# xdspacelab/openvslam

Measured on AMD Instinct MI355X. Metric: ORB kpts+descriptors/sec and Hamming matches/sec @1920x1080, 8-level pyramid, higher is better.
Workload: dtype u8; 1 GPU; BASELINE configs[1]: 1920x1080 mono, 8 pyramid levels (x1.2), 2000 ORB features, extract + robust::brute_force_match (thr 50, ratio 0.9) against the previous frame; distinct_input_batches=2

## Files before the change

openvslam_amd/csrc/orb_describe.hip:

```cpp
#include <cstdlib>

#include "ovs_common.h"

namespace ovs {

__constant__ int8_t c_pattern[256 * 4] = {
#include "orb_pattern.inc"
};
__constant__ int32_t c_umax[16] = {15, 15, 15, 15, 14, 14, 14, 13, 13, 12, 11, 10, 9, 8, 6, 3};
__constant__ uint32_t c_ic_tab[16 * 2 * 8] = {
    0x01010100u, 0x01010101u, 0x01010101u, 0x01010101u, 0x03020100u, 0x07060504u, 0x0b0a0908u, 0x0f0e0d0cu,
    0x01010101u, 0x01010101u, 0x01010101u, 0x01010101u, 0x13121110u, 0x17161514u, 0x1b1a1918u, 0x1f1e1d1cu,
    0x01010100u, 0x01010101u, 0x01010101u, 0x01010101u, 0x03020100u, 0x07060504u, 0x0b0a0908u, 0x0f0e0d0cu,
    0x01010101u, 0x01010101u, 0x01010101u, 0x01010101u, 0x13121110u, 0x17161514u, 0x1b1a1918u, 0x1f1e1d1cu,
    0x01010100u, 0x01010101u, 0x01010101u, 0x01010101u, 0x03020100u, 0x07060504u, 0x0b0a0908u, 0x0f0e0d0cu,
    0x01010101u, 0x01010101u, 0x01010101u, 0x01010101u, 0x13121110u, 0x17161514u, 0x1b1a1918u, 0x1f1e1d1cu,
    0x01010100u, 0x01010101u, 0x01010101u, 0x01010101u, 0x03020100u, 0x07060504u, 0x0b0a0908u, 0x0f0e0d0cu,
    0x01010101u, 0x01010101u, 0x01010101u, 0x01010101u, 0x13121110u, 0x17161514u, 0x1b1a1918u, 0x1f1e1d1cu,
    0x01010000u, 0x01010101u, 0x01010101u, 0x01010101u, 0x03020000u, 0x07060504u, 0x0b0a0908u, 0x0f0e0d0cu,
    0x01010101u, 0x01010101u, 0x01010101u, 0x00010101u, 0x13121110u, 0x17161514u, 0x1b1a1918u, 0x001e1d1cu,
    0x01010000u, 0x01010101u, 0x01010101u, 0x01010101u, 0x03020000u, 0x07060504u, 0x0b0a0908u, 0x0f0e0d0cu,
    0x01010101u, 0x01010101u, 0x01010101u, 0x00010101u, 0x13121110u, 0x17161514u, 0x1b1a1918u, 0x001e1d1cu,
    0x01010000u, 0x01010101u, 0x01010101u, 0x01010101u, 0x03020000u, 0x07060504u, 0x0b0a0908u, 0x0f0e0d0cu,
    0x01010101u, 0x01010101u, 0x01010101u, 0x00010101u, 0x13121110u, 0x17161514u, 0x1b1a1918u, 0x001e1d1cu,
    0x01000000u, 0x01010101u, 0x01010101u, 0x01010101u, 0x03000000u, 0x07060504u, 0x0b0a0908u, 0x0f0e0d0cu,
    0x01010101u, 0x01010101u, 0x01010101u, 0x00000101u, 0x13121110u, 0x17161514u, 0x1b1a1918u, 0x00001d1cu,
    0x01000000u, 0x01010101u, 0x01010101u, 0x01010101u, 0x03000000u, 0x07060504u, 0x0b0a0908u, 0x0f0e0d0cu,
    0x01010101u, 0x01010101u, 0x01010101u, 0x00000101u, 0x13121110u, 0x17161514u, 0x1b1a1918u, 0x00001d1cu,
    0x00000000u, 0x01010101u, 0x01010101u, 0x01010101u, 0x00000000u, 0x07060504u, 0x0b0a0908u, 0x0f0e0d0cu,
    0x01010101u, 0x01010101u, 0x01010101u, 0x00000001u, 0x13121110u, 0x17161514u, 0x1b1a1918u, 0x0000001cu,
    0x00000000u, 0x01010100u, 0x01010101u, 0x01010101u, 0x00000000u, 0x07060500u, 0x0b0a0908u, 0x0f0e0d0cu,
    0x01010101u, 0x01010101u, 0x01010101u, 0x00000000u, 0x13121110u, 0x17161514u, 0x1b1a1918u, 0x00000000u,
    0x00000000u, 0x01010000u, 0x01010101u, 0x01010101u, 0x00000000u, 0x07060000u, 0x0b0a0908u, 0x0f0e0d0cu,
    0x01010101u, 0x01010101u, 0x00010101u, 0x00000000u, 0x13121110u, 0x17161514u, 0x001a1918u, 0x00000000u,
    0x00000000u, 0x01000000u, 0x01010101u, 0x01010101u, 0x00000000u, 0x07000000u, 0x0b0a0908u, 0x0f0e0d0cu,
    0x01010101u, 0x01010101u, 0x00000101u, 0x00000000u, 0x13121110u, 0x17161514u, 0x00001918u, 0x00000000u,
    0x00000000u, 0x00000000u, 0x01010101u, 0x01010101u, 0x00000000u, 0x00000000u, 0x0b0a0908u, 0x0f0e0d0cu,
    0x01010101u, 0x01010101u, 0x00000001u, 0x00000000u, 0x13121110u, 0x17161514u, 0x00000018u, 0x00000000u,
    0x00000000u, 0x00000000u, 0x01010000u, 0x01010101u, 0x00000000u, 0x00000000u, 0x0b0a0000u, 0x0f0e0d0cu,
    0x01010101u, 0x00010101u, 0x00000000u, 0x00000000u, 0x13121110u, 0x00161514u, 0x00000000u, 0x00000000u,
    0x00000000u, 0x00000000u, 0x00000000u, 0x01010100u, 0x00000000u, 0x00000000u, 0x00000000u, 0x0f0e0d00u,
    0x01010101u, 0x00000000u, 0x00000000u, 0x00000000u, 0x13121110u, 0x00000000u, 0x00000000u, 0x00000000u,
};
constexpr uint32_t kG0123 = 18u | (34u << 8) | (48u << 16) | (56u << 24);
constexpr uint32_t kG456 = 48u | (34u << 8) | (18u << 16);
constexpr uint32_t kG0123Indep = 18u | (34u << 8) | (49u << 16) | (55u << 24);
constexpr uint32_t kG456Indep = 49u | (34u << 8) | (18u << 16);

constexpr int kPatch = 43;
constexpr int kPatchR = 21;
constexpr int kBlurW = 37;
constexpr int kBlurR = 18;
constexpr int kPatchPitch = 64;
constexpr int kHbPitch = 40;
static_assert(kBlurW <= kHbPitch && kBlurW + 6 == kPatch, "blur window geometry");

__device__ __forceinline__ float fast_atan2_deg(float y, float x) {
    const float p1 = 0.9997878412794807f * (float)(180 / 3.14159265358979323846);
    const float p3 = -0.3258083974640975f * (float)(180 / 3.14159265358979323846);
    const float p5 = 0.1555786518463281f * (float)(180 / 3.14159265358979323846);
    const float p7 = -0.04432655554792128f * (float)(180 / 3.14159265358979323846);
    const float eps = 2.2204460492503131e-16f;
    const float ax = fabsf(x), ay = fabsf(y);
    float a, c, c2;
    if (ax >= ay) {
        c = __fdiv_rn(ay, __fadd_rn(ax, eps));
        c2 = __fmul_rn(c, c);
        a = __fmul_rn(__fadd_rn(__fmul_rn(__fadd_rn(__fmul_rn(__fadd_rn(__fmul_rn(p7, c2), p5), c2), p3), c2), p1), c);
    } else {
        c = __fdiv_rn(ax, __fadd_rn(ay, eps));
        c2 = __fmul_rn(c, c);
        a = __fsub_rn(90.f, __fmul_rn(__fadd_rn(__fmul_rn(__fadd_rn(__fmul_rn(__fadd_rn(__fmul_rn(p7, c2), p5), c2), p3), c2), p1), c));
    }
    if (x < 0) a = __fsub_rn(180.f, a);
    if (y < 0) a = __fsub_rn(360.f, a);
    return a;
}

__device__ __forceinline__ float poly_cos(float v) {
    const float c1 = 0.99940307f, c2 = -0.49558072f, c3 = 0.03679168f;
    const float v2 = __fmul_rn(v, v);
    return __fadd_rn(c1, __fmul_rn(v2, __fadd_rn(c2, __fmul_rn(c3, v2))));
}
__device__ __forceinline__ float util_cos(float v) {
    const float kPi = 3.14159265358979323846f, kTwoPi = 6.28318530717958647692f, kHalfPi = 1.57079632679489661923f,
                kThreeHalfPi = 4.71238898038468985769f, kInvTwoPi = 0.15915494309189533577f;
    v = __fsub_rn(v, __fmul_rn(floorf(__fmul_rn(v, kInvTwoPi)), kTwoPi));
    v = (0.0f < v) ? v : -v;
    if (v < kHalfPi) return poly_cos(v);
    if (v < kPi) return -poly_cos(__fsub_rn(kPi, v));
    if (v < kThreeHalfPi) return -poly_cos(__fsub_rn(v, kPi));
    return poly_cos(__fsub_rn(kTwoPi, v));
}
__device__ __forceinline__ float util_sin(float v) { return util_cos(__fsub_rn(1.57079632679489661923f, v)); }

template <int BYTE>
__device__ __forceinline__ float cvt_s8(uint32_t w) {
    float f;
    if (BYTE == 0) asm("v_cvt_f32_i32_sdwa %0, sext(%1) dst_sel:DWORD dst_unused:UNUSED_PAD src0_sel:BYTE_0" : "=v"(f) : "v"(w));
    if (BYTE == 1) asm("v_cvt_f32_i32_sdwa %0, sext(%1) dst_sel:DWORD dst_unused:UNUSED_PAD src0_sel:BYTE_1" : "=v"(f) : "v"(w));
    if (BYTE == 2) asm("v_cvt_f32_i32_sdwa %0, sext(%1) dst_sel:DWORD dst_unused:UNUSED_PAD src0_sel:BYTE_2" : "=v"(f) : "v"(w));
    if (BYTE == 3) asm("v_cvt_f32_i32_sdwa %0, sext(%1) dst_sel:DWORD dst_unused:UNUSED_PAD src0_sel:BYTE_3" : "=v"(f) : "v"(w));
    return f;
}

__device__ __forceinline__ int wave_total_in_lane63(int v) {
    v += __builtin_amdgcn_update_dpp(0, v, 0x111, 0xf, 0xf, true);
    v += __builtin_amdgcn_update_dpp(0, v, 0x112, 0xf, 0xf, true);
    v += __builtin_amdgcn_update_dpp(0, v, 0x114, 0xf, 0xf, true);
    v += __builtin_amdgcn_update_dpp(0, v, 0x118, 0xf, 0xf, true);
    v += __builtin_amdgcn_update_dpp(0, v, 0x142, 0xa, 0xf, false);
    v += __builtin_amdgcn_update_dpp(0, v, 0x143, 0xc, 0xf, false);
    return v;
}

__global__ __launch_bounds__(64) void k_describe(const FrameGeo* __restrict__ geo, const uint8_t* __restrict__ img0, size_t stride0,
                                                size_t frame_stride0, const uint8_t* __restrict__ pyr, size_t pyr_frame_bytes,
                                                const uint64_t* __restrict__ lvl_kps, const uint32_t* __restrict__ lvl_count,
                                                ovs_keypoint* __restrict__ kps, uint8_t* __restrict__ desc,
                                                int32_t* __restrict__ counts, int cap, int batch, ovs_keypoint* __restrict__ kps_m,
                                                uint8_t* __restrict__ desc_m, int32_t* __restrict__ counts_m) {
    __shared__ __attribute__((aligned(16))) uint8_t patch[kPatch * kPatchPitch];
    __shared__ __attribute__((aligned(16))) uint16_t hblur[kPatch * kHbPitch];

    const int lane = threadIdx.x;
    const int total_cap = geo->total_kp_cap;
    const uint32_t xcd = blockIdx.x & 7u, idx = blockIdx.x >> 3;
    const uint32_t grp = idx / (uint32_t)total_cap;
    const int kslot = (int)(idx - grp * (uint32_t)total_cap);
    const int frame = (int)(grp * 8u + xcd);
    if (frame >= batch) return;
    const int L = geo->num_levels;
    int level = 0;
    for (int l = 1; l < L; ++l)
        if (kslot >= geo->lv[l].kp_base) level = l;
    const LevelGeo& g = geo->lv[level];
    const int slot = kslot - g.kp_base;
    const uint32_t* cnt = lvl_count + frame * L;
    if (kslot == 0 && lane == 0) {
        int total = 0;
        for (int l = 0; l < L; ++l) total += cnt[l];
        counts[frame] = total < cap ? total : cap;
        if (counts_m) counts_m[frame] = total < cap ? total : cap;
    }
    if (slot >= (int)cnt[level]) return;
    int out_idx = slot;
    for (int l = 0; l < level; ++l) out_idx += cnt[l];
    if (out_idx >= cap) return;

    const uint64_t kp = lvl_kps[(size_t)frame * total_cap + kslot];
    const int x = (int)cand_x(kp), y = (int)cand_y(kp);
    const uint8_t* img;
    int pitch;
    if (level == 0) {
        img = img0 + (size_t)frame * frame_stride0;
        pitch = (int)stride0;
    } else {
        img = pyr + (size_t)frame * pyr_frame_bytes + g.plane_off;
        pitch = g.pitch;
    }
    const int xs = x - kPatchR;
    const int xa = xs & ~15;
    const int off = __builtin_amdgcn_readfirstlane(xs - xa);
    const uint8_t* seg0 = img + (size_t)(y - kPatchR) * pitch + xa;
    if (((pitch & 15) == 0) && ((reinterpret_cast<uintptr_t>(img) & 15) == 0)) {
#pragma unroll
        for (int j = 0; j < 3; ++j) {
            const int i = lane + 64 * j;
            if (i < kPatch * 4) {
                const int r = i >> 2, q = i & 3;
                *reinterpret_cast<uint4*>(patch + r * kPatchPitch + 16 * q) = *reinterpret_cast<const uint4*>(seg0 + (size_t)r * pitch + 16 * q);
            }
        }
    } else {
        for (int i = lane; i < kPatch * 16; i += 64) {
            const int r = i >> 4, q = i & 15;
            *reinterpret_cast<uint32_t*>(patch + r * kPatchPitch + 4 * q) = *reinterpret_cast<const uint32_t*>(seg0 + (size_t)r * pitch + 4 * q);
        }
    }
    __syncthreads();

    int m10 = 0, m01 = 0;
    if (lane < 62) {
        const int v = (lane >> 1) - 15, h = lane & 1;
        const int first = off + kPatchR + (h ? 0 : -16);
        const uint32_t* pw = reinterpret_cast<const uint32_t*>(patch + (kPatchR + v) * kPatchPitch + (first & ~3));
        const int shb = first & 3;
        const uint32_t w0 = pw[0], w1 = pw[1], w2 = pw[2], w3 = pw[3], w4 = pw[4];
        const uint32_t px[4] = {__builtin_amdgcn_alignbyte(w1, w0, shb), __builtin_amdgcn_alignbyte(w2, w1, shb),
                                __builtin_amdgcn_alignbyte(w3, w2, shb), __builtin_amdgcn_alignbyte(w4, w3, shb)};
        const uint32_t* tab = c_ic_tab + (((v < 0 ? -v : v) * 2 + h) << 3);
        uint32_t sum = 0, wsum = 0;
#pragma unroll
        for (int q = 0; q < 4; ++q) {
            sum = __builtin_amdgcn_udot4(px[q], tab[q], sum, false);
            wsum = __builtin_amdgcn_udot4(px[q], tab[4 + q], wsum, false);
        }
        m10 = (int)wsum - 16 * (int)sum;
        m01 = v * (int)sum;
    }
    m10 = __builtin_amdgcn_readlane(wave_total_in_lane63(m10), 63);
    m01 = __builtin_amdgcn_readlane(wave_total_in_lane63(m01), 63);
    const float angle = fast_atan2_deg((float)m01, (float)m10);
    const float rad = ovs_det_deg2rad(angle);
    const bool trig_libm = (geo->variant & 8) != 0;
    const float cos_a = trig_libm ? ovs_det_cosf(rad) : util_cos(rad), sin_a = trig_libm ? ovs_det_sinf(rad) : util_sin(rad);

    const int sh = off & 3;
    const bool taps_indep = (geo->variant & 4) != 0;
    const uint32_t g0123 = taps_indep ? kG0123Indep : kG0123, g456 = taps_indep ? kG456Indep : kG456;
    uint32_t* hb32 = reinterpret_cast<uint32_t*>(hblur);
    const unsigned long long taps = (unsigned long long)g0123 | ((unsigned long long)g456 << 32);
    const uint32_t t1a = (uint32_t)(taps << 8), t1b = (uint32_t)(taps >> 24);
    const uint32_t t2a = (uint32_t)(taps << 16), t2b = (uint32_t)(taps >> 16), t2c = (uint32_t)(taps >> 48);
    const uint32_t t3a = (uint32_t)(taps << 24), t3b = (uint32_t)(taps >> 8), t3c = (uint32_t)(taps >> 40);
    if (lane < 60) {
        const int r0 = (lane * 0x199a) >> 16, q = lane - 10 * r0;
        const uint32_t* const pw0 = reinterpret_cast<const uint32_t*>(patch + r0 * kPatchPitch + ((off + 4 * q) & ~3));
        uint32_t* const hb0 = hb32 + r0 * (kHbPitch / 2) + 2 * q;
#pragma unroll
        for (int it = 0; it < 8; ++it) {
            if (it == 7 && r0 != 0) break;
            const uint32_t* pw = pw0 + it * 6 * (kPatchPitch / 4);
            const uint32_t w0 = pw[0], w1 = pw[1], w2 = pw[2], w3 = pw[3];
            const uint32_t n0 = __builtin_amdgcn_alignbyte(w1, w0, sh), n1 = __builtin_amdgcn_alignbyte(w2, w1, sh),
                           n2 = __builtin_amdgcn_alignbyte(w3, w2, sh);
            const uint32_t o0 = __builtin_amdgcn_udot4(n0, g0123, __builtin_amdgcn_udot4(n1, g456, 0u, false), false);
            const uint32_t o1 = __builtin_amdgcn_udot4(n0, t1a, __builtin_amdgcn_udot4(n1, t1b, 0u, false), false);
            const uint32_t o2 = __builtin_amdgcn_udot4(n0, t2a, __builtin_amdgcn_udot4(n1, t2b, __builtin_amdgcn_udot4(n2, t2c, 0u, false), false), false);
            const uint32_t o3 = __builtin_amdgcn_udot4(n0, t3a, __builtin_amdgcn_udot4(n1, t3b, __builtin_amdgcn_udot4(n2, t3c, 0u, false), false), false);
            uint32_t* hb = hb0 + it * 6 * (kHbPitch / 2);
            hb[0] = o0 | (o1 << 16);
            hb[1] = o2 | (o3 << 16);
        }
    }
    __syncthreads();

    auto blurred_at = [&](float fx, float fy) -> int {
        const int dy = __float2int_rn(__fadd_rn(__fmul_rn(fx, sin_a), __fmul_rn(fy, cos_a)));
        const int dx = __float2int_rn(__fsub_rn(__fmul_rn(fx, cos_a), __fmul_rn(fy, sin_a)));
        const uint16_t* hp = hblur + (dy + kBlurR) * kHbPitch + dx + kBlurR;
        const uint32_t a0 = (uint32_t)hp[0] + hp[6 * kHbPitch], a1 = (uint32_t)hp[kHbPitch] + hp[5 * kHbPitch],
                       a2 = (uint32_t)hp[2 * kHbPitch] + hp[4 * kHbPitch], a3 = hp[3 * kHbPitch];
        uint32_t acc = 32768u;
        acc += (g0123 & 255u) * a0;
        acc += ((g0123 >> 8) & 255u) * a1;
        acc += ((g0123 >> 16) & 255u) * a2;
        acc += (g0123 >> 24) * a3;
        return (int)min(acc >> 16, 255u);
    };
    unsigned long long bits[4];
    const uint32_t* pat = reinterpret_cast<const uint32_t*>(c_pattern);
#pragma unroll
    for (int t = 0; t < 4; ++t) {
        const uint32_t pp = pat[lane + 64 * t];
        const int t0 = blurred_at(cvt_s8<0>(pp), cvt_s8<1>(pp));
        const int t1 = blurred_at(cvt_s8<2>(pp), cvt_s8<3>(pp));
        bits[t] = __ballot(t0 < t1);
    }
    if (lane < 4) {
        const unsigned long long b = lane == 0 ? bits[0] : lane == 1 ? bits[1] : lane == 2 ? bits[2] : bits[3];
        reinterpret_cast<unsigned long long*>(desc + ((size_t)frame * cap + out_idx) * 32)[lane] = b;
        if (desc_m) reinterpret_cast<unsigned long long*>(desc_m + ((size_t)frame * cap + out_idx) * 32)[lane] = b;
    }
    if (lane == 0) {
        ovs_keypoint k;
        k.x = __fmul_rn((float)x, g.scale);
        k.y = __fmul_rn((float)y, g.scale);
        k.size = g.kp_size;
        k.angle = angle;
        k.response = (float)cand_score(kp);
        k.octave = level;
        k.class_id = -1;
        kps[(size_t)frame * cap + out_idx] = k;
        if (kps_m) kps_m[(size_t)frame * cap + out_idx] = k;
    }
}

hipError_t launch_describe(const FrameGeo& hgeo, const DevBuffers& d, const uint8_t* img0, size_t stride0, size_t frame_stride0,
                           ovs_keypoint* kps, uint8_t* desc, int32_t* counts, int cap, int batch, hipStream_t s, ovs_keypoint* kps_m, uint8_t* desc_m,
                           int32_t* counts_m) {
    const int frames = (batch + 7) & ~7;
    dim3 grid((unsigned)hgeo.total_kp_cap * (unsigned)frames);
    hipLaunchKernelGGL(k_describe, grid, dim3(64), 0, s, d.geo, img0, stride0, frame_stride0, d.pyr, d.pyr_frame_bytes, d.lvl_kps,
                       d.lvl_count, kps, desc, counts, cap, batch, kps_m, desc_m, counts_m);
    return hipGetLastError();
}

}
```

Baseline: 160.0 million keypoints+descriptors/s.

## Describe two keypoints per wavefront with half-wave split in ORB descriptor kernel

Adds a k_describe_pair kernel in which each 64-lane block handles two keypoints, one per 32-lane half. Each half stages its own patch in shared memory, runs the moment, blur and descriptor stages, and uses half-wave DPP reductions and ballot splits. This halves the number of blocks and is meant to raise lane utilisation over the old one-keypoint-per-wave path. It also swaps the branchy cos and atan2 for select-based versions. The new path runs only when batch>1 and no mirror outputs are requested, and per-lane work (32 rather than 64 lanes) is denser, which may add register pressure.

```diff
diff --git a/openvslam_amd/csrc/orb_describe.hip b/openvslam_amd/csrc/orb_describe.hip
--- a/openvslam_amd/csrc/orb_describe.hip
+++ b/openvslam_amd/csrc/orb_describe.hip
@@ -94,6 +94,31 @@
 }
 __device__ __forceinline__ float util_sin(float v) { return util_cos(__fsub_rn(1.57079632679489661923f, v)); }
 
+__device__ __forceinline__ float fast_atan2_deg_sel(float y, float x) {
+    const float p1 = 0.9997878412794807f * (float)(180 / 3.14159265358979323846);
+    const float p3 = -0.3258083974640975f * (float)(180 / 3.14159265358979323846);
+    const float p5 = 0.1555786518463281f * (float)(180 / 3.14159265358979323846);
+    const float p7 = -0.04432655554792128f * (float)(180 / 3.14159265358979323846);
+    const float eps = 2.2204460492503131e-16f;
+    const float ax = fabsf(x), ay = fabsf(y);
+    const bool xs = ax >= ay;
+    const float c = __fdiv_rn(xs ? ay : ax, __fadd_rn(xs ? ax : ay, eps));
+    const float c2 = __fmul_rn(c, c);
+    const float p = __fmul_rn(__fadd_rn(__fmul_rn(__fadd_rn(__fmul_rn(__fadd_rn(__fmul_rn(p7, c2), p5), c2), p3), c2), p1), c);
+    float a = xs ? p : __fsub_rn(90.f, p);
+    a = x < 0 ? __fsub_rn(180.f, a) : a;
+    return y < 0 ? __fsub_rn(360.f, a) : a;
+}
+__device__ __forceinline__ float util_cos_sel(float v) {
+    const float kPi = 3.14159265358979323846f, kTwoPi = 6.28318530717958647692f, kHalfPi = 1.57079632679489661923f,
+                kThreeHalfPi = 4.71238898038468985769f, kInvTwoPi = 0.15915494309189533577f;
+    v = __fsub_rn(v, __fmul_rn(floorf(__fmul_rn(v, kInvTwoPi)), kTwoPi));
+    v = (0.0f < v) ? v : -v;
+    const float r = v < kHalfPi ? v : v < kPi ? __fsub_rn(kPi, v) : v < kThreeHalfPi ? __fsub_rn(v, kPi) : __fsub_rn(kTwoPi, v);
+    const float p = poly_cos(r);
+    return (v < kHalfPi || !(v < kThreeHalfPi)) ? p : -p;
+}
+
 template <int BYTE>
 __device__ __forceinline__ float cvt_s8(uint32_t w) {
     float f;
@@ -277,10 +302,198 @@
     }
 }
 
+constexpr int kTilePitch = 2 * kHbPitch;
+__global__ __launch_bounds__(64) void k_describe_pair(const FrameGeo* __restrict__ geo, const uint8_t* __restrict__ img0, size_t stride0,
+                                                     size_t frame_stride0, const uint8_t* __restrict__ pyr, size_t pyr_frame_bytes,
+                                                     const uint64_t* __restrict__ lvl_kps, const uint32_t* __restrict__ lvl_count,
+                                                     ovs_keypoint* __restrict__ kps, uint8_t* __restrict__ desc, int32_t* __restrict__ counts,
+                                                     int cap, int batch, int pairs_per_frame) {
+    __shared__ __attribute__((aligned(16))) uint16_t hblur[2 * kPatch * kHbPitch];
+
+    const int lane = threadIdx.x, half = lane >> 5, hl = lane & 31;
+    const uint32_t xcd = blockIdx.x & 7u, idx = blockIdx.x >> 3;
+    const uint32_t grp = idx / (uint32_t)pairs_per_frame;
+    const int pidx = (int)(idx - grp * (uint32_t)pairs_per_frame);
+    const int frame = (int)(grp * 8u + xcd);
+    if (frame >= batch) return;
+    const int L = geo->num_levels;
+    const uint32_t* cnt = lvl_count + frame * L;
+    if (pidx == 0 && lane == 0) {
+        int total = 0;
+        for (int l = 0; l < L; ++l) total += cnt[l];
+        counts[frame] = total < cap ? total : cap;
+    }
+    int level = 0, pbase = 0, out_base = 0;
+    for (int l = 0; l + 1 < L; ++l) {
+        const int np = (geo->lv[l].kp_cap + 1) >> 1;
+        if (pidx < pbase + np) break;
+        pbase += np;
+        out_base += (int)cnt[l];
+        level = l + 1;
+    }
+    const LevelGeo& g = geo->lv[level];
+    const int slot0 = 2 * (pidx - pbase);
+    const int n = (int)cnt[level];
+    if (slot0 >= n || out_base + slot0 >= cap) return;
+    const bool valid = slot0 + half < n && out_base + slot0 + half < cap;
+    const int slot = valid ? slot0 + half : slot0;
+    const int out_idx = out_base + slot;
+
+    const uint64_t kp = lvl_kps[(size_t)frame * geo->total_kp_cap + g.kp_base + slot];
+    const int x = (int)cand_x(kp), y = (int)cand_y(kp);
+    const uint8_t* img;
+    int pitch;
+    if (level == 0) {
+        img = img0 + (size_t)frame * frame_stride0;
+        pitch = (int)stride0;
+    } else {
+        img = pyr + (size_t)frame * pyr_frame_bytes + g.plane_off;
+        pitch = g.pitch;
+    }
+    const int xs = x - kPatchR;
+    const int xa = xs & ~15;
+    const int off = xs - xa;
+    const uint8_t* seg0 = img + (size_t)(y - kPatchR) * pitch + xa;
+    uint8_t* const mypatch = reinterpret_cast<uint8_t*>(hblur + half * (kPatch * kHbPitch));
+    if (((pitch & 15) == 0) && ((reinterpret_cast<uintptr_t>(img) & 15) == 0)) {
+#pragma unroll
+        for (int j = 0; j < 6; ++j) {
+            const int i = hl + 32 * j;
+            if (i < kPatch * 4) {
+                const int r = i >> 2, q = i & 3;
+                *reinterpret_cast<uint4*>(mypatch + r * kTilePitch + 16 * q) = *reinterpret_cast<const uint4*>(seg0 + (size_t)r * pitch + 16 * q);
+            }
+        }
+    } else {
+        for (int i = hl; i < kPatch * 16; i += 32) {
+            const int r = i >> 4, q = i & 15;
+            *reinterpret_cast<uint32_t*>(mypatch + r * kTilePitch + 4 * q) = *reinterpret_cast<const uint32_t*>(seg0 + (size_t)r * pitch + 4 * q);
+        }
+    }
+    __syncthreads();
+
+    int m10 = 0, m01 = 0;
+#pragma unroll
+    for (int s = 0; s < 2; ++s) {
+        const int task = hl + 32 * s;
+        if (task < 62) {
+            const int v = (task >> 1) - 15, h = task & 1;
+            const int first = off + kPatchR + (h ? 0 : -16);
+            const uint32_t* pw = reinterpret_cast<const uint32_t*>(mypatch + (kPatchR + v) * kTilePitch + (first & ~3));
+            const int shb = first & 3;
+            const uint32_t w0 = pw[0], w1 = pw[1], w2 = pw[2], w3 = pw[3], w4 = pw[4];
+            const uint32_t px[4] = {__builtin_amdgcn_alignbyte(w1, w0, shb), __builtin_amdgcn_alignbyte(w2, w1, shb),
+                                    __builtin_amdgcn_alignbyte(w3, w2, shb), __builtin_amdgcn_alignbyte(w4, w3, shb)};
+            const uint32_t* tab = c_ic_tab + (((v < 0 ? -v : v) * 2 + h) << 3);
+            uint32_t sum = 0, wsum = 0;
+#pragma unroll
+            for (int q = 0; q < 4; ++q) {
+                sum = __builtin_amdgcn_udot4(px[q], tab[q], sum, false);
+                wsum = __builtin_amdgcn_udot4(px[q], tab[4 + q], wsum, false);
+            }
+            m10 += (int)wsum - 16 * (int)sum;
+            m01 += v * (int)sum;
+        }
+    }
+    auto half_total = [half](int v) {
+        v += __builtin_amdgcn_update_dpp(0, v, 0x111, 0xf, 0xf, true);
+        v += __builtin_amdgcn_update_dpp(0, v, 0x112, 0xf, 0xf, true);
+        v += __builtin_amdgcn_update_dpp(0, v, 0x114, 0xf, 0xf, true);
+        v += __builtin_amdgcn_update_dpp(0, v, 0x118, 0xf, 0xf, true);
+        v += __builtin_amdgcn_update_dpp(0, v, 0x142, 0xa, 0xf, false);
+        const int lo = __builtin_amdgcn_readlane(v, 31), hi = __builtin_amdgcn_readlane(v, 63);
+        return half ? hi : lo;
+    };
+    m10 = half_total(m10);
+    m01 = half_total(m01);
+    const float angle = fast_atan2_deg_sel((float)m01, (float)m10);
+    const float rad = ovs_det_deg2rad(angle);
+    const bool trig_libm = (geo->variant & 8) != 0;
+    const float cos_a = trig_libm ? ovs_det_cosf(rad) : util_cos_sel(rad);
+    const float sin_a = trig_libm ? ovs_det_sinf(rad) : util_cos_sel(__fsub_rn(1.57079632679489661923f, rad));
+
+    const int sh = off & 3;
+    const bool taps_indep = (geo->variant & 4) != 0;
+    const uint32_t g0123 = taps_indep ? kG0123Indep : kG0123, g456 = taps_indep ? kG456Indep : kG456;
+    const unsigned long long taps = (unsigned long long)g0123 | ((unsigned long long)g456 << 32);
+    const uint32_t t1a = (uint32_t)(taps << 8), t1b = (uint32_t)(taps >> 24);
+    const uint32_t t2a = (uint32_t)(taps << 16), t2b = (uint32_t)(taps >> 16), t2c = (uint32_t)(taps >> 48);
+    const uint32_t t3a = (uint32_t)(taps << 24), t3b = (uint32_t)(taps >> 8), t3c = (uint32_t)(taps >> 40);
+    uint16_t* const myblur = hblur + half * (kPatch * kHbPitch);
+    if (hl < 30) {
+        const int r0 = (hl * 0x199a) >> 16, q = hl - 10 * r0;
+        const uint32_t* const pw0 = reinterpret_cast<const uint32_t*>(mypatch + r0 * kTilePitch + ((off + 4 * q) & ~3));
+        uint32_t* const hb0 = reinterpret_cast<uint32_t*>(myblur) + r0 * (kHbPitch / 2) + 2 * q;
+#pragma unroll
+        for (int it = 0; it < 15; ++it) {
+            if (it == 14 && r0 != 0) break;
+            const uint32_t* pw = pw0 + it * 3 * (kTilePitch / 4);
+            const uint32_t w0 = pw[0], w1 = pw[1], w2 = pw[2], w3 = pw[3];
+            const uint32_t n0 = __builtin_amdgcn_alignbyte(w1, w0, sh), n1 = __builtin_amdgcn_alignbyte(w2, w1, sh),
+                           n2 = __builtin_amdgcn_alignbyte(w3, w2, sh);
+            const uint32_t o0 = __builtin_amdgcn_udot4(n0, g0123, __builtin_amdgcn_udot4(n1, g456, 0u, false), false);
+            const uint32_t o1 = __builtin_amdgcn_udot4(n0, t1a, __builtin_amdgcn_udot4(n1, t1b, 0u, false), false);
+            const uint32_t o2 = __builtin_amdgcn_udot4(n0, t2a, __builtin_amdgcn_udot4(n1, t2b, __builtin_amdgcn_udot4(n2, t2c, 0u, false), false), false);
+            const uint32_t o3 = __builtin_amdgcn_udot4(n0, t3a, __builtin_amdgcn_udot4(n1, t3b, __builtin_amdgcn_udot4(n2, t3c, 0u, false), false), false);
+            uint32_t* hb = hb0 + it * 3 * (kHbPitch / 2);
+            hb[0] = o0 | (o1 << 16);
+            hb[1] = o2 | (o3 << 16);
+        }
+    }
+    __syncthreads();
+
+    constexpr float kRound = 12582912.0f;
+    const uint32_t hb_base = (uint32_t)half * (2u * kPatch * kHbPitch) + 2u * (kBlurR * kHbPitch + kBlurR);
+    const uint32_t kHbAdj = hb_base - 0x400000u * (2u * kHbPitch) - 2u * __float_as_uint(kRound);
+    const uint8_t* const hb8 = reinterpret_cast<const uint8_t*>(hblur);
+    auto blurred_at = [&](float fx, float fy) -> int {
+        const uint32_t by = __float_as_uint(__fadd_rn(__fadd_rn(__fmul_rn(fx, sin_a), __fmul_rn(fy, cos_a)), kRound));
+        const uint32_t bx = __float_as_uint(__fadd_rn(__fsub_rn(__fmul_rn(fx, cos_a), __fmul_rn(fy, sin_a)), kRound));
+        const uint16_t* hp = reinterpret_cast<const uint16_t*>(hb8 + (__umul24(by, 2u * kHbPitch) + 2u * bx + kHbAdj));
+        const uint32_t a0 = (uint32_t)hp[0] + hp[6 * kHbPitch], a1 = (uint32_t)hp[kHbPitch] + hp[5 * kHbPitch],
+                       a2 = (uint32_t)hp[2 * kHbPitch] + hp[4 * kHbPitch], a3 = hp[3 * kHbPitch];
+        uint32_t acc = 32768u;
+        acc += (g0123 & 255u) * a0;
+        acc += ((g0123 >> 8) & 255u) * a1;
+        acc += ((g0123 >> 16) & 255u) * a2;
+        acc += (g0123 >> 24) * a3;
+        return (int)min(acc >> 16, 255u);
+    };
+    uint32_t word = 0;
+    const uint32_t* pat = reinterpret_cast<const uint32_t*>(c_pattern);
+#pragma unroll
+    for (int t = 0; t < 8; ++t) {
+        const uint32_t pp = pat[hl + 32 * t];
+        const int t0 = blurred_at(cvt_s8<0>(pp), cvt_s8<1>(pp));
+        const int t1 = blurred_at(cvt_s8<2>(pp), cvt_s8<3>(pp));
+        const unsigned long long b = __ballot(t0 < t1);
+        if (hl == t) word = half ? (uint32_t)(b >> 32) : (uint32_t)b;
+    }
+    if (valid && hl < 8) reinterpret_cast<uint32_t*>(desc + ((size_t)frame * cap + out_idx) * 32)[hl] = word;
+    if (valid && hl == 0) {
+        ovs_keypoint k;
+        k.x = __fmul_rn((float)x, g.scale);
+        k.y = __fmul_rn((float)y, g.scale);
+        k.size = g.kp_size;
+        k.angle = angle;
+        k.response = (float)cand_score(kp);
+        k.octave = level;
+        k.class_id = -1;
+        kps[(size_t)frame * cap + out_idx] = k;
+    }
+}
+
 hipError_t launch_describe(const FrameGeo& hgeo, const DevBuffers& d, const uint8_t* img0, size_t stride0, size_t frame_stride0,
                            ovs_keypoint* kps, uint8_t* desc, int32_t* counts, int cap, int batch, hipStream_t s, ovs_keypoint* kps_m, uint8_t* desc_m,
                            int32_t* counts_m) {
     const int frames = (batch + 7) & ~7;
+    if (batch > 1 && !kps_m && !desc_m && !counts_m) {
+        int pairs = 0;
+        for (int l = 0; l < hgeo.num_levels; ++l) pairs += (hgeo.lv[l].kp_cap + 1) >> 1;
+        hipLaunchKernelGGL(k_describe_pair, dim3((unsigned)pairs * (unsigned)frames), dim3(64), 0, s, d.geo, img0, stride0, frame_stride0, d.pyr,
+                           d.pyr_frame_bytes, d.lvl_kps, d.lvl_count, kps, desc, counts, cap, batch, pairs);
+        return hipGetLastError();
+    }
     dim3 grid((unsigned)hgeo.total_kp_cap * (unsigned)frames);
     hipLaunchKernelGGL(k_describe, grid, dim3(64), 0, s, d.geo, img0, stride0, frame_stride0, d.pyr, d.pyr_frame_bytes, d.lvl_kps,
                        d.lvl_count, kps, desc, counts, cap, batch, kps_m, desc_m, counts_m);
```

Result: faster. 161.7 million keypoints+descriptors/s (median of 6 runs) (+1.1%).
